# PaddlePaddle/Parakeet

Hardware: NVIDIA H100
Metric: audio-samples/sec (higher is better)
Workload: dtype bf16x3 (split-bf16 operands, fp32 accumulate; fp32-grade, 1e-3 parity)

## Files before the change

### parakeet_b200/csrc/pwg.cu

```cuda
#include <stdlib.h>
#include <string.h>

#include <algorithm>

#include "pk_host.h"
#include "pk_sm90.cuh"

namespace pk {

constexpr int kPwgR = 64;
constexpr int kPwgG = 128;
constexpr int kPwgS = 64;
constexpr int kPwgStages = 2;
constexpr int kPwgTile = 128 * kSwizzleBytes;
constexpr int kPwgStageBytes = 4 * kPwgTile;
constexpr int kPwgW2Bytes = 2 * kPwgTile;
constexpr int kPwgSmem = kPwgStages * kPwgStageBytes + kPwgW2Bytes + 1024 + 256;
static_assert(kPwgSmem <= 227 * 1024, "shared memory budget");
constexpr int kPwgConsumerThreads = 256;
constexpr int kPwgThreads = kPwgConsumerThreads + 128;
constexpr int kPwgG1Chunks = 5;

struct PwgLayerArgs {
  int batch, t, dil, aux_ch;
// ... 353 lines not shown
      }
      if (c_hi) {
        uint4 h, l;
        split8(v, h, l);
        const long long o = (static_cast<long long>(b) * T + t) * aux + g * 8;
        *reinterpret_cast<uint4*>(c_hi + o) = h;
        *reinterpret_cast<uint4*>(c_lo + o) = l;
      }
    }
  }
}

__global__ void pwg_first_conv_kernel(const float* __restrict__ noise, const float* __restrict__ w, const float* __restrict__ bias,
                                      const int32_t* __restrict__ lens, int t_len, long long total_rows,
                                      __nv_bfloat16* __restrict__ x_hi, __nv_bfloat16* __restrict__ x_lo) {
  const long long n = total_rows * 8;
  for (long long idx = blockIdx.x * static_cast<long long>(blockDim.x) + threadIdx.x; idx < n;
       idx += static_cast<long long>(gridDim.x) * blockDim.x) {
    const long long row = idx >> 3;
    const int g = idx & 7;
    const int b = row / t_len, t = row % t_len;
    const bool live = lens == nullptr || t < __ldg(lens + b);
    const float xv = __ldg(noise + row);
    float v[8];
#pragma unroll
    for (int e = 0; e < 8; ++e) v[e] = live ? fmaf(__ldg(w + g * 8 + e), xv, __ldg(bias + g * 8 + e)) : 0.f;
    uint4 h, l;
    split8(v, h, l);
    reinterpret_cast<uint4*>(x_hi)[idx] = h;
    reinterpret_cast<uint4*>(x_lo)[idx] = l;
  }
}

__global__ void __launch_bounds__(128)
pwg_tail_kernel(const float* __restrict__ skip, const float* __restrict__ skip_bias ,
                const float* __restrict__ w1 , const float* __restrict__ b1,
                const float* __restrict__ w2 , const float* __restrict__ b2, float scale, long long rows,
                float* __restrict__ out) {
  __shared__ float4 sw1[16 * 64];
  __shared__ float sb1[64], sw2[64], ssb[64];
  for (int i = threadIdx.x; i < 64 * 16; i += blockDim.x) {
    const int o = i >> 4, kq = i & 15;
    sw1[kq * 64 + o] = reinterpret_cast<const float4*>(w1)[i];
  }
  if (threadIdx.x < 64) {
    sb1[threadIdx.x] = b1[threadIdx.x];
    sw2[threadIdx.x] = w2[threadIdx.x];
    ssb[threadIdx.x] = skip_bias ? skip_bias[threadIdx.x] : 0.f;
  }
  __syncthreads();
  const float bias2 = __ldg(b2);
  const long long pairs = (rows + 1) >> 1;
  for (long long pr = blockIdx.x * static_cast<long long>(blockDim.x) + threadIdx.x; pr < pairs;
       pr += static_cast<long long>(gridDim.x) * blockDim.x) {
    const long long r0 = pr, r1 = pr + pairs;
    const bool has1 = r1 < rows;
    const float4* p0 = reinterpret_cast<const float4*>(skip + r0 * 64);
    const float4* p1 = reinterpret_cast<const float4*>(skip + (has1 ? r1 : r0) * 64);
    float h0[64], h1[64];
#pragma unroll
    for (int o = 0; o < 64; ++o) { h0[o] = sb1[o]; h1[o] = sb1[o]; }
#pragma unroll 1
    for (int kc = 0; kc < 4; ++kc) {
      float s0[16], s1[16];
#pragma unroll
      for (int q = 0; q < 4; ++q) {
        const float4 u = __ldg(p0 + kc * 4 + q), v = __ldg(p1 + kc * 4 + q);
        const float* sbp = ssb + kc * 16 + q * 4;
        s0[4 * q] = fmaxf((u.x + sbp[0]) * scale, 0.f); s0[4 * q + 1] = fmaxf((u.y + sbp[1]) * scale, 0.f);
        s0[4 * q + 2] = fmaxf((u.z + sbp[2]) * scale, 0.f); s0[4 * q + 3] = fmaxf((u.w + sbp[3]) * scale, 0.f);
        s1[4 * q] = fmaxf((v.x + sbp[0]) * scale, 0.f); s1[4 * q + 1] = fmaxf((v.y + sbp[1]) * scale, 0.f);
        s1[4 * q + 2] = fmaxf((v.z + sbp[2]) * scale, 0.f); s1[4 * q + 3] = fmaxf((v.w + sbp[3]) * scale, 0.f);
      }
#pragma unroll
      for (int q = 0; q < 4; ++q) {
#pragma unroll
        for (int o = 0; o < 64; ++o) {
          const float4 w = sw1[(kc * 4 + q) * 64 + o];
          h0[o] = fmaf(w.x, s0[4 * q], h0[o]); h0[o] = fmaf(w.y, s0[4 * q + 1], h0[o]);
          h0[o] = fmaf(w.z, s0[4 * q + 2], h0[o]); h0[o] = fmaf(w.w, s0[4 * q + 3], h0[o]);
          h1[o] = fmaf(w.x, s1[4 * q], h1[o]); h1[o] = fmaf(w.y, s1[4 * q + 1], h1[o]);
          h1[o] = fmaf(w.z, s1[4 * q + 2], h1[o]); h1[o] = fmaf(w.w, s1[4 * q + 3], h1[o]);
        }
      }
    }
    float y0 = bias2, y1 = bias2;
#pragma unroll
    for (int o = 0; o < 64; ++o) {
      y0 = fmaf(sw2[o], fmaxf(h0[o], 0.f), y0);
      y1 = fmaf(sw2[o], fmaxf(h1[o], 0.f), y1);
    }
    out[r0] = y0;
    if (has1) out[r1] = y1;
  }
}

}

extern "C" int pk_pwg_residual_layer(const pk_pwg_layer_args* a, pk_stream_t stream) {
  PK_CHECK_ARG(a != nullptr, "args is NULL");
// ... 93 lines not shown
  const size_t smem = floats * sizeof(float);
  PK_CHECK_ARG(smem <= 200 * 1024, "upsample tile does not fit shared memory (%zu bytes)", smem);
  static size_t attr_smem = 0;
  if (smem > attr_smem) {
    PK_CHECK_CUDA(cudaFuncSetAttribute(pwg_upsample_kernel, cudaFuncAttributeMaxDynamicSharedMemorySize, static_cast<int>(smem)));
    attr_smem = smem;
  }
  dim3 grid(frames, batch);
  pwg_upsample_kernel<<<grid, 256, smem, st>>>(conv_in_ws, frame_lens, a, c_f32, static_cast<__nv_bfloat16*>(c_hi),
                                               static_cast<__nv_bfloat16*>(c_lo));
  PK_CHECK_CUDA(cudaGetLastError());
  count_launch();
  return PK_OK;
}

extern "C" int pk_pwg_first_conv(const float* noise, const float* w, const float* bias, const int32_t* lens, int32_t batch,
                                 int32_t t, void* x_hi, void* x_lo, pk_stream_t stream) {
  PK_CHECK_ARG(noise && w && bias && x_hi && x_lo, "NULL pointer");
  PK_CHECK_ARG(batch > 0 && t > 0, "bad sizes");
  const long long rows = static_cast<long long>(batch) * t;
  const int threads = 256;
  const int blocks = static_cast<int>(std::min<long long>((rows * 8 + threads - 1) / threads, pk::sm_count() * 16LL));
  pk::pwg_first_conv_kernel<<<blocks, threads, 0, static_cast<cudaStream_t>(stream)>>>(
      noise, w, bias, lens, t, rows, static_cast<__nv_bfloat16*>(x_hi), static_cast<__nv_bfloat16*>(x_lo));
  PK_CHECK_CUDA(cudaGetLastError());
  pk::count_launch();
  return PK_OK;
}

extern "C" int pk_pwg_tail(const float* skip, const float* skip_bias, const float* w1, const float* b1, const float* w2,
                           const float* b2, float scale, int64_t rows, float* out, pk_stream_t stream) {
  PK_CHECK_ARG(skip && w1 && b1 && w2 && b2 && out, "NULL pointer");
  PK_CHECK_ARG(rows > 0, "bad sizes");
  const int threads = 128;
  const long long pairs = (rows + 1) / 2;
  const int blocks = static_cast<int>(std::min<long long>((pairs + threads - 1) / threads, pk::sm_count() * 12LL));
  pk::pwg_tail_kernel<<<blocks, threads, 0, static_cast<cudaStream_t>(stream)>>>(skip, skip_bias, w1, b1, w2, b2, scale, rows, out);
  PK_CHECK_CUDA(cudaGetLastError());
  pk::count_launch();
  return PK_OK;
}
```

### parakeet_b200/csrc/pk_sm90.cuh

```cuda
#pragma once
#include <cuda.h>
#include <cuda_bf16.h>
#include <cuda_runtime.h>
#include <stdint.h>

namespace pk {

constexpr int kSwizzleBytes = 128;
constexpr int kChunkK = 64;

__device__ __forceinline__ uint32_t smem_u32(const void* p) {
  return static_cast<uint32_t>(__cvta_generic_to_shared(p));
}

__device__ __forceinline__ void fence_barrier_init() {
  asm volatile("fence.mbarrier_init.release.cluster;" ::: "memory");
}

__device__ __forceinline__ void fence_proxy_async_all() { asm volatile("fence.proxy.async;" ::: "memory"); }

__device__ __forceinline__ void tma_prefetch_desc(const CUtensorMap* tm) {
  asm volatile("prefetch.tensormap [%0];" ::"l"(reinterpret_cast<uint64_t>(tm)) : "memory");
}

constexpr int kWgmmaK = 16;

__device__ __forceinline__ uint64_t make_smem_desc_sw128(uint32_t smem_addr) {
  uint64_t d = 0;
  d |= static_cast<uint64_t>((smem_addr & 0x3FFFFu) >> 4);
  d |= static_cast<uint64_t>(1) << 16;
  d |= static_cast<uint64_t>(1024 >> 4) << 32;
  d |= static_cast<uint64_t>(1) << 62;
  return d;
}
__device__ __forceinline__ uint64_t desc_kstep(int k) { return static_cast<uint64_t>((k * kWgmmaK * 2) >> 4); }
__device__ __forceinline__ uint64_t make_smem_desc_sw32(uint32_t smem_addr) {
  uint64_t d = 0;
  d |= static_cast<uint64_t>((smem_addr & 0x3FFFFu) >> 4);
  d |= static_cast<uint64_t>(1) << 16;
  d |= static_cast<uint64_t>(256 >> 4) << 32;
  d |= static_cast<uint64_t>(3) << 62;
  return d;
}

__device__ __forceinline__ void wgmma_fence() { asm volatile("wgmma.fence.sync.aligned;" ::: "memory"); }
__device__ __forceinline__ void wgmma_commit() { asm volatile("wgmma.commit_group.sync.aligned;" ::: "memory"); }
template <int N>
__device__ __forceinline__ void wgmma_wait() { asm volatile("wgmma.wait_group.sync.aligned %0;" ::"n"(N) : "memory"); }
template <int R>
__device__ __forceinline__ void reg_fence(float (&d)[R]) {
#pragma unroll
  for (int i = 0; i < R; ++i) asm volatile("" : "+f"(d[i])::"memory");
// ... 44 lines not shown
  asm volatile("{\n.reg .pred p;\nsetp.ne.b32 p, %101, 0;\n"
               "wgmma.mma_async.sync.aligned.m64n192k16.f32.bf16.bf16 {" PK_D96 "}, {%96,%97,%98,%99}, %100, p, 1, 1, 0;\n}\n"
               : PK_F32(0), PK_F32(32), PK_F32(64) : "r"(a[0]), "r"(a[1]), "r"(a[2]), "r"(a[3]), "l"(bdesc), "r"(accumulate));
}
#undef PK_F32
#undef PK_F8

__device__ __forceinline__ void split_bf16(float v, __nv_bfloat16& hi, __nv_bfloat16& lo) {
  hi = __float2bfloat16_rn(v);
  lo = __float2bfloat16_rn(v - __bfloat162float(hi));
}
__device__ __forceinline__ uint32_t pack_bf16x2(__nv_bfloat16 a, __nv_bfloat16 b) {
  return static_cast<uint32_t>(__bfloat16_as_ushort(a)) | (static_cast<uint32_t>(__bfloat16_as_ushort(b)) << 16);
}
__device__ __forceinline__ void split8(const float* v, uint4& hi, uint4& lo) {
  __nv_bfloat16 h[8], l[8];
#pragma unroll
  for (int i = 0; i < 8; ++i) split_bf16(v[i], h[i], l[i]);
  hi = make_uint4(pack_bf16x2(h[0], h[1]), pack_bf16x2(h[2], h[3]), pack_bf16x2(h[4], h[5]), pack_bf16x2(h[6], h[7]));
  lo = make_uint4(pack_bf16x2(l[0], l[1]), pack_bf16x2(l[2], l[3]), pack_bf16x2(l[4], l[5]), pack_bf16x2(l[6], l[7]));
}


__device__ __forceinline__ float4 lds_f4(uint32_t addr) {
  float4 v;
  asm volatile("ld.shared.v4.f32 {%0, %1, %2, %3}, [%4];" : "=f"(v.x), "=f"(v.y), "=f"(v.z), "=f"(v.w) : "r"(addr));
  return v;
}
__device__ __forceinline__ uint32_t lds_u32(uint32_t addr) {
  uint32_t v;
  asm volatile("ld.shared.u32 %0, [%1];" : "=r"(v) : "r"(addr) : "memory");
  return v;
}
__device__ __forceinline__ void sts_u32(uint32_t addr, uint32_t v) {
  asm volatile("st.shared.u32 [%0], %1;" ::"r"(addr), "r"(v) : "memory");
}

__device__ __forceinline__ void mbar_init_a(uint32_t bar, uint32_t count) {
  asm volatile("mbarrier.init.shared::cta.b64 [%0], %1;" ::"r"(bar), "r"(count) : "memory");
}
__device__ __forceinline__ void mbar_arrive_expect_tx_a(uint32_t bar, uint32_t bytes) {
  asm volatile("mbarrier.arrive.expect_tx.shared::cta.b64 _, [%0], %1;" ::"r"(bar), "r"(bytes) : "memory");
}
__device__ __forceinline__ void mbar_arrive_a(uint32_t bar) {
  asm volatile("mbarrier.arrive.shared::cta.b64 _, [%0];" ::"r"(bar) : "memory");
}
__device__ __forceinline__ void mbar_wait_a(uint32_t bar, uint32_t parity) {
  uint32_t ok = 0;
  for (uint32_t spin = 0; spin < (1u << 26); ++spin) {
    asm volatile(
        "{\n"
        ".reg .pred p;\n"
        "mbarrier.try_wait.parity.shared::cta.b64 p, [%1], %2;\n"
        "selp.u32 %0, 1, 0, p;\n"
        "}\n"
        : "=r"(ok)
        : "r"(bar), "r"(parity)
        : "memory");
    if (ok) return;
  }
  __trap();
}
__device__ __forceinline__ void tma_load_3d_a(uint32_t smem_dst, const CUtensorMap* tm, uint32_t bar, int c0, int c1, int c2) {
  asm volatile(
      "cp.async.bulk.tensor.3d.shared::cluster.global.tile.mbarrier::complete_tx::bytes [%0], [%1, {%3, %4, %5}], [%2];"
      ::"r"(smem_dst), "l"(reinterpret_cast<uint64_t>(tm)), "r"(bar), "r"(c0), "r"(c1), "r"(c2)
      : "memory");
}
__device__ __forceinline__ void tma_load_4d_a(uint32_t smem_dst, const CUtensorMap* tm, uint32_t bar, int c0, int c1, int c2, int c3) {
  asm volatile(
      "cp.async.bulk.tensor.4d.shared::cluster.global.tile.mbarrier::complete_tx::bytes [%0], [%1, {%3, %4, %5, %6}], [%2];"
      ::"r"(smem_dst), "l"(reinterpret_cast<uint64_t>(tm)), "r"(bar), "r"(c0), "r"(c1), "r"(c2), "r"(c3)
      : "memory");
}
__device__ __forceinline__ void tma_store_4d_a(const CUtensorMap* tm, uint32_t smem_src, int c0, int c1, int c2, int c3) {
  asm volatile("cp.async.bulk.tensor.4d.global.shared::cta.bulk_group [%0, {%2, %3, %4, %5}], [%1];"
               ::"l"(reinterpret_cast<uint64_t>(tm)), "r"(smem_src), "r"(c0), "r"(c1), "r"(c2), "r"(c3)
               : "memory");
}
__device__ __forceinline__ void bulk_prefetch_l2(const void* gptr, uint32_t bytes) {
  asm volatile("cp.async.bulk.prefetch.L2.global [%0], %1;" ::"l"(reinterpret_cast<uint64_t>(gptr)), "r"(bytes) : "memory");
}
__device__ __forceinline__ void bulk_commit() { asm volatile("cp.async.bulk.commit_group;" ::: "memory"); }
template <int N>
__device__ __forceinline__ void bulk_wait_read() { asm volatile("cp.async.bulk.wait_group.read %0;" ::"n"(N) : "memory"); }


constexpr int kStageSlotBytes = 64 * 32 * 4;
__device__ __forceinline__ uint32_t stage_addr(uint32_t slot, int row, int col) {
  return slot + row * 128 + ((((col >> 2) ^ (row & 7)) << 4) | ((col & 3) << 2));
}
template <int R>
__device__ __forceinline__ void stage_store(uint32_t slot, const float (&d)[R], int C, int wg_thread) {
  const int w = wg_thread >> 5, lane = wg_thread & 31;
  const int r0 = 16 * w + (lane >> 2), c0 = 2 * (lane & 3);
#pragma unroll
  for (int jj = 0; jj < 4; ++jj) {
    const int j = 4 * C + jj;
    asm volatile("st.shared.v2.f32 [%0], {%1, %2};" ::"r"(stage_addr(slot, r0, 8 * jj + c0)), "f"(d[4 * j]), "f"(d[4 * j + 1]) : "memory");
    asm volatile("st.shared.v2.f32 [%0], {%1, %2};" ::"r"(stage_addr(slot, r0 + 8, 8 * jj + c0)), "f"(d[4 * j + 2]), "f"(d[4 * j + 3])
                 : "memory");
  }
}
__device__ __forceinline__ void stage_load_row(uint32_t slot, int row, float (&v)[32]) {
#pragma unroll
  for (int k = 0; k < 8; ++k) {
    const float4 x = lds_f4(slot + row * 128 + ((k ^ (row & 7)) << 4));
    v[4 * k] = x.x; v[4 * k + 1] = x.y; v[4 * k + 2] = x.z; v[4 * k + 3] = x.w;
  }
}

}
```

### parakeet_b200/csrc/pwg_fc.cu

```cuda
#include <stdlib.h>
#include <string.h>

#include <algorithm>

#include "pk_host.h"
#include "pk_sm90.cuh"

namespace pk {
namespace fc {

constexpr int kPwgR = 64;
constexpr int kPwgG = 128;
constexpr int kATile = 128 * kSwizzleBytes;
constexpr int kQTile = 64 * kSwizzleBytes;
constexpr int kConsumerThreads = 256;
constexpr int kThreads = kConsumerThreads + 128;
constexpr int kFcG1Chunks = 4;
constexpr int kFcStages = 6;
constexpr int kFcStageBytes = 2 * kQTile;
constexpr int kFcUBytes = 2 * 64 * 32;
constexpr int kFcPBytes = 2 * 128 * 32;
constexpr int kFcW1Bytes = 3 * 2 * kATile;
constexpr int kFcW2Bytes = 2 * kATile;
constexpr int kFcSmem = kFcW1Bytes + kFcW2Bytes + kFcStages * kFcStageBytes + 1024 + 256;
static_assert(kFcUBytes + kFcPBytes <= kFcStageBytes, "the conditioning operands share one ring stage");
static_assert(kFcSmem <= 227 * 1024, "shared memory budget");

struct FcLayerArgs {
  int batch, t, dil, hop;
  int u_period, u_start_row, u_end_base;
  int p_row0;
  const int32_t* lens;
  float gate_c[128];
  float out_b[64];
  float k_a, k_g;
  float* skip;
  int skip_init;
};

__device__ __forceinline__ float ex2_approx(float x) {
  float y;
  asm("ex2.approx.ftz.f32 %0, %1;" : "=f"(y) : "f"(x));
  return y;
}
__device__ __forceinline__ float rcp_approx(float x) {
  float y;
  asm("rcp.approx.ftz.f32 %0, %1;" : "=f"(y) : "f"(x));
  return y;
}
__device__ __forceinline__ void split2(float a, float b, uint32_t& hi, uint32_t& lo) {
  const __nv_bfloat162 h = __floats2bfloat162_rn(a, b);
  hi = *reinterpret_cast<const uint32_t*>(&h);
  const float ra = a - __uint_as_float(hi << 16);
  const float rb = b - __uint_as_float(hi & 0xffff0000u);
  const __nv_bfloat162 l = __floats2bfloat162_rn(ra, rb);
  lo = *reinterpret_cast<const uint32_t*>(&l);
}

struct FcTileIter {
  int idx, step, tiles_per_b, total, t;
  const int32_t* lens;
  __device__ FcTileIter(const FcLayerArgs& p)
      : idx(static_cast<int>(blockIdx.x) - static_cast<int>(gridDim.x)), step(gridDim.x),
        tiles_per_b((p.t + 255) >> 8), total(((p.t + 255) >> 8) * p.batch * 2), t(p.t), lens(p.lens) {}
  __device__ bool next(int& b, int& m0, int& half) {
    for (;;) {
      idx += step;
      if (idx >= total) return false;
      const int w = idx >> 1;
      half = idx & 1;
      b = w / tiles_per_b;
      m0 = (w % tiles_per_b) * 256;
      const int len = lens ? min(__ldg(lens + b), t) : t;
      if (m0 < len) return true;
    }
  }
};

__global__ void __launch_bounds__(kThreads, 1)
pwg_layer_fc_kernel(const __grid_constant__ CUtensorMap tm_x, const __grid_constant__ CUtensorMap tm_u,
                    const __grid_constant__ CUtensorMap tm_p,
                    const __grid_constant__ CUtensorMap tm_w1_hi, const __grid_constant__ CUtensorMap tm_w1_lo,
                    const __grid_constant__ CUtensorMap tm_w2_hi, const __grid_constant__ CUtensorMap tm_w2_lo,
                    const __grid_constant__ CUtensorMap tm_y, const FcLayerArgs p) {
  extern __shared__ uint8_t smem_raw[];
  const uint32_t smem = (smem_u32(smem_raw) + 1023u) & ~1023u;
  const uint32_t w1 = smem;
  const uint32_t w2 = w1 + kFcW1Bytes;
  const uint32_t ring = w2 + kFcW2Bytes;
  const uint32_t bars = ring + kFcStages * kFcStageBytes;
  const uint32_t full_bar = bars;
  const uint32_t empty_bar = full_bar + 8 * kFcStages;
  const uint32_t w_bar = empty_bar + 8 * kFcStages;

  const int warp = threadIdx.x >> 5;
  const int lane = threadIdx.x & 31;

  if (threadIdx.x == kConsumerThreads) {
    tma_prefetch_desc(&tm_x); tma_prefetch_desc(&tm_u); tma_prefetch_desc(&tm_p);
    tma_prefetch_desc(&tm_w1_hi); tma_prefetch_desc(&tm_w1_lo); tma_prefetch_desc(&tm_w2_hi); tma_prefetch_desc(&tm_w2_lo);
    tma_prefetch_desc(&tm_y);
    for (int s = 0; s < kFcStages; ++s) { mbar_init_a(full_bar + 8 * s, 1); mbar_init_a(empty_bar + 8 * s, 4); }
    mbar_init_a(w_bar, 1);
    fence_barrier_init();
  }
  __syncthreads();

  if (warp >= kConsumerThreads / 32) {
    setmaxnreg_dec<40>();
    if (warp == kConsumerThreads / 32 && lane == 0) {
      mbar_arrive_expect_tx_a(w_bar, kFcW1Bytes + kFcW2Bytes);
      for (int j = 0; j < 3; ++j) {
        tma_load_3d_a(w1 + j * 2 * kATile, &tm_w1_hi, w_bar, j * kChunkK, 0, 0);
        tma_load_3d_a(w1 + j * 2 * kATile + kATile, &tm_w1_lo, w_bar, j * kChunkK, 0, 0);
      }
      tma_load_3d_a(w2, &tm_w2_hi, w_bar, 0, 0, 0);
      tma_load_3d_a(w2 + kATile, &tm_w2_lo, w_bar, 0, 0, 0);
      uint32_t it = 0;
      FcTileIter ti(p);
      int b, m0, half;
      while (ti.next(b, m0, half)) {
        const int mh = m0 + 128 * half;
        const int len = p.lens ? min(__ldg(p.lens + b), p.t) : p.t;
        const int m1 = ((len - 128) >> 7) << 7;
        const int urow = mh == 0 ? p.u_start_row
                         : (mh + 128 > len - 128) ? p.u_end_base + 384 * b + min(mh - m1, 256)
                                                  : mh % p.u_period;
        const int j0 = (m0 / p.hop - 2) & ~7;
        for (int wg = 0; wg < 2; ++wg) {
          const int rows = min(64, p.t - (mh + 64 * wg));
          if (!p.skip_init && rows > 0)
            bulk_prefetch_l2(p.skip + (static_cast<long long>(b) * p.t + mh + 64 * wg) * 64, rows * 64 * 4);
          for (int j = 0; j < kFcG1Chunks; ++j, ++it) {
            const int s = it % kFcStages;
            mbar_wait_a(empty_bar + 8 * s, ((it / kFcStages) & 1) ^ 1);
            const uint32_t st = ring + s * kFcStageBytes;
            const uint32_t fb = full_bar + 8 * s;
            if (j == 2) {
              mbar_arrive_expect_tx_a(fb, kFcUBytes + kFcPBytes);
              tma_load_4d_a(st, &tm_u, fb, 0, urow + 64 * wg, 0, 0);
              tma_load_4d_a(st + kFcUBytes, &tm_p, fb, j0, p.p_row0, b, 0);
            } else {
              mbar_arrive_expect_tx_a(fb, kFcStageBytes);
              const int wj = j == 0 ? 0 : j == 1 ? 2 : 1;
              tma_load_4d_a(st, &tm_x, fb, 0, mh + 64 * wg + (wj - 1) * p.dil, b, 0);
            }
          }
        }
      }
    }
  } else {
    setmaxnreg_inc<232>();
    const int wg = warp >> 2;
    const int rl = 16 * (warp & 3) + (lane >> 2);
    const int cq = 2 * (lane & 3);
    const float kSqrtHalf = 0.70710678118654752440f;
    mbar_wait_a(w_bar, 0);
    uint32_t it = wg * kFcG1Chunks;
    FcTileIter ti(p);
    int b, m0, half;
    bool more = ti.next(b, m0, half);
    bool first = true;
    while (more) {
      const int mh = m0 + 128 * half;
      float acc1[64], acc2[64];
      if (wg == 1 || !first) named_bar_sync(1 + wg, kConsumerThreads);
      first = false;
#pragma unroll
      for (int j = 0; j < kFcG1Chunks; ++j) {
        const int s = (it + j) % kFcStages;
        mbar_wait_a(full_bar + 8 * s, ((it + j) / kFcStages) & 1);
        const uint32_t st = ring + s * kFcStageBytes;
        wgmma_fence();
        if (j == 2) {
          const uint64_t a_hi = make_smem_desc_sw32(st), a_lo = make_smem_desc_sw32(st + kFcUBytes / 2);
          const uint64_t b_hi = make_smem_desc_sw32(st + kFcUBytes), b_lo = make_smem_desc_sw32(st + kFcUBytes + kFcPBytes / 2);
          wgmma_ss_n128(acc1, a_hi, b_hi, 1);
          wgmma_ss_n128(acc1, a_lo, b_hi, 1);
          wgmma_ss_n128(acc1, a_hi, b_lo, 1);
        } else {
          const int wj = j == 0 ? 0 : j == 1 ? 2 : 1;
          const uint64_t a_hi = make_smem_desc_sw128(st), a_lo = make_smem_desc_sw128(st + kQTile);
          const uint64_t b_hi = make_smem_desc_sw128(w1 + wj * 2 * kATile), b_lo = make_smem_desc_sw128(w1 + wj * 2 * kATile + kATile);
#pragma unroll
          for (int k = 0; k < 4; ++k) {
            wgmma_ss_n128(acc1, a_hi + desc_kstep(k), b_hi + desc_kstep(k), !(j == 0 && k == 0));
            wgmma_ss_n128(acc1, a_lo + desc_kstep(k), b_hi + desc_kstep(k), 1);
            wgmma_ss_n128(acc1, a_hi + desc_kstep(k), b_lo + desc_kstep(k), 1);
          }
        }
        wgmma_commit();
        if (j == kFcG1Chunks - 1) {
#pragma unroll
          for (int jj = 0; jj < 8; ++jj) {
#pragma unroll
            for (int hh = 0; hh < 2; ++hh) {
              const int r = rl + 8 * hh;
              const uint32_t off = r * kSwizzleBytes + ((((8 * jj + cq) >> 3) ^ (r & 7)) << 4) + (cq & 7) * 2;
              const uint32_t xh = lds_u32(st + off), xl = lds_u32(st + kQTile + off);
              acc2[4 * jj + 2 * hh] = 0.f;
              acc2[4 * jj + 2 * hh + 1] = 0.f;
              acc2[32 + 4 * jj + 2 * hh] = __uint_as_float(xh << 16) + __uint_as_float(xl << 16);
              acc2[32 + 4 * jj + 2 * hh + 1] = __uint_as_float(xh & 0xffff0000u) + __uint_as_float(xl & 0xffff0000u);
            }
          }
        }
        if (j > 0) {
          wgmma_wait<1>();
          __syncwarp();
          if (lane == 0) mbar_arrive_a(empty_bar + 8 * ((it + j - 1) % kFcStages));
        }
      }
      wgmma_wait<0>();
      reg_fence(acc1);
      const int cs = (it + kFcG1Chunks - 1) % kFcStages;
      const uint32_t ystage = ring + cs * kFcStageBytes;
      it += 2 * kFcG1Chunks;
      int nb, nm0, nhalf;
      const bool next = ti.next(nb, nm0, nhalf);
      if (wg == 0 || next) named_bar_arrive(2 - wg, kConsumerThreads);
      uint32_t zh[16], zl[16];
#pragma unroll
      for (int jj = 0; jj < 8; ++jj) {
        float z[4];
#pragma unroll
        for (int e = 0; e < 4; ++e) {
          const int c = 8 * jj + cq + (e & 1);
          const float e1 = ex2_approx(fminf(fmaf(acc1[4 * jj + e], p.k_a, p.gate_c[c]), 60.f));
          const float e2 = ex2_approx(fmaf(acc1[32 + 4 * jj + e], p.k_g, p.gate_c[64 + c]));
          const float t1 = 1.f + e1;
          z[e] = (1.f - e1) * rcp_approx(fmaf(t1, e2, t1));
        }
        split2(z[0], z[1], zh[2 * jj], zl[2 * jj]);
        split2(z[2], z[3], zh[2 * jj + 1], zl[2 * jj + 1]);
      }
      const uint64_t b2_hi = make_smem_desc_sw128(w2), b2_lo = make_smem_desc_sw128(w2 + kATile);
      wgmma_fence();
#pragma unroll
      for (int k = 0; k < 4; ++k) {
        const uint32_t ah[4] = {zh[4 * k], zh[4 * k + 1], zh[4 * k + 2], zh[4 * k + 3]};
        const uint32_t al[4] = {zl[4 * k], zl[4 * k + 1], zl[4 * k + 2], zl[4 * k + 3]};
        wgmma_rs_n128(acc2, ah, b2_hi + desc_kstep(k), 1);
        wgmma_rs_n128(acc2, al, b2_hi + desc_kstep(k), 1);
        wgmma_rs_n128(acc2, ah, b2_lo + desc_kstep(k), 1);
      }
      wgmma_commit();
      wgmma_wait<0>();
      reg_fence(acc2);
      const int len = p.lens ? min(__ldg(p.lens + b), p.t) : p.t;
#pragma unroll
      for (int hh = 0; hh < 2; ++hh) {
        const int r = rl + 8 * hh;
        const bool live = mh + wg * 64 + r < len;
#pragma unroll
        for (int jj = 0; jj < 8; ++jj) {
          const int c = 8 * jj + cq;
          const float y0 = live ? (acc2[32 + 4 * jj + 2 * hh] + p.out_b[c]) * kSqrtHalf : 0.f;
          const float y1 = live ? (acc2[32 + 4 * jj + 2 * hh + 1] + p.out_b[c + 1]) * kSqrtHalf : 0.f;
          uint32_t oh, ol;
          split2(y0, y1, oh, ol);
          const uint32_t off = r * kSwizzleBytes + (((c >> 3) ^ (r & 7)) << 4) + (cq & 7) * 2;
          sts_u32(ystage + off, oh);
          sts_u32(ystage + kQTile + off, ol);
        }
      }
      fence_proxy_async_all();
      named_bar_sync(3 + wg, 128);
      const bool store_lane = (threadIdx.x & 127) == 0;
      if (store_lane) {
        tma_store_4d_a(&tm_y, ystage, 0, mh + wg * 64, b, 0);
        bulk_commit();
      }
#pragma unroll
      for (int hh = 0; hh < 2; ++hh) {
        const int trow = mh + wg * 64 + rl + 8 * hh;
        if (trow < p.t) {
          const long long row_off = (static_cast<long long>(b) * p.t + trow) * 64;
#pragma unroll
          for (int jj = 0; jj < 8; ++jj) {
            float* d2 = p.skip + row_off + 8 * jj + cq;
            const float s0 = acc2[4 * jj + 2 * hh], s1 = acc2[4 * jj + 2 * hh + 1];
            if (p.skip_init) *reinterpret_cast<float2*>(d2) = make_float2(s0, s1);
            else asm volatile("red.global.add.v2.f32 [%0], {%1, %2};" ::"l"(d2), "f"(s0), "f"(s1) : "memory");
          }
        }
      }
      if (store_lane) {
        bulk_wait_read<0>();
#pragma unroll
        for (int w = 0; w < 4; ++w) mbar_arrive_a(empty_bar + 8 * cs);
      }
      b = nb; m0 = nm0; half = nhalf; more = next;
    }
  }
}

}
}

extern "C" int pk_pwg_residual_layer_fc(const pk_pwg_layer_fc_args* a, pk_stream_t stream) {
  using namespace pk;
  using namespace pk::fc;
  PK_CHECK_ARG(a != nullptr, "args is NULL");
  PK_CHECK_ARG(a->batch > 0 && a->t > 0 && a->dilation >= 1 && a->hop >= 256, "bad batch/t/dilation/hop (hop must be >= 256)");
  PK_CHECK_ARG(a->x_hi && a->x_lo && a->y_hi && a->y_lo && a->u_hi && a->u_lo && a->p_hi && a->p_lo && a->w1_hi && a->w1_lo &&
               a->w2_hi && a->w2_lo && a->bias1 && a->bias2 && a->skip, "NULL pointer in pk_pwg_layer_fc_args");
  PK_CHECK_ARG(a->x_hi != a->y_hi, "layer output must not alias its input");
  PK_CHECK_ARG(a->u_period > 0 && (a->u_period % 128) == 0 && a->u_start_row >= a->u_period && a->u_end_base >= a->u_start_row + 128 &&
               a->u_rows >= a->u_end_base + 384 * a->batch, "bad compact band table layout");
  PK_CHECK_ARG(a->p_rows > 0 && a->p_row0 >= 0 && a->p_row0 + 128 <= a->p_rows && (a->p_ld % 8) == 0 && a->p_ld >= 64 && a->p_frames > 0 &&
               a->p_frames <= a->p_ld, "bad P plane geometry");
  CUtensorMap tx, tu, tp, tw1_hi, tw1_lo, tw2_hi, tw2_lo, ty;
  int rc;
  const uint64_t T = a->t, B = a->batch;
  if ((rc = encode_tmap_bf16_planes(&tx, a->x_hi, a->x_lo, kPwgR, T, B, kPwgR, T * kPwgR, 64))) return rc;
  if ((rc = encode_tmap_bf16_planes(&ty, a->y_hi, a->y_lo, kPwgR, T, B, kPwgR, T * kPwgR, 64))) return rc;
  if ((rc = encode_tmap_bf16_planes(&tu, a->u_hi, a->u_lo, 64, a->u_rows, 1, 64, 0, 64, 16))) return rc;
  const uint64_t prow = a->p_rows, pld = a->p_ld;
  if ((rc = encode_tmap_bf16_planes(&tp, a->p_hi, a->p_lo, pld, prow, B, pld, prow * pld, 128, 16))) return rc;
  const uint64_t k1 = 5 * kChunkK;
  if ((rc = encode_tmap_bf16_3d(&tw1_hi, a->w1_hi, 3 * kChunkK, kPwgG, 1, k1, k1 * kPwgG, 128))) return rc;
  if ((rc = encode_tmap_bf16_3d(&tw1_lo, a->w1_lo, 3 * kChunkK, kPwgG, 1, k1, k1 * kPwgG, 128))) return rc;
  if ((rc = encode_tmap_bf16_3d(&tw2_hi, a->w2_hi, 64, 128, 1, 64, 0, 128))) return rc;
  if ((rc = encode_tmap_bf16_3d(&tw2_lo, a->w2_lo, 64, 128, 1, 64, 0, 128))) return rc;
  static bool attr_set = false;
  if (!attr_set) {
    PK_CHECK_CUDA(cudaFuncSetAttribute(pwg_layer_fc_kernel, cudaFuncAttributeMaxDynamicSharedMemorySize, kFcSmem));
    attr_set = true;
  }
  FcLayerArgs p;
  p.batch = a->batch; p.t = a->t; p.dil = a->dilation; p.hop = a->hop;
  p.u_period = a->u_period; p.u_start_row = a->u_start_row; p.u_end_base = a->u_end_base;
  p.p_row0 = a->p_row0;
  p.lens = a->lens; p.skip = a->skip; p.skip_init = a->skip_init;
  constexpr float kLog2e = 1.4426950408889634f;
  p.k_a = -2.f * kLog2e; p.k_g = -kLog2e;
  for (int i = 0; i < 64; ++i) {
    p.gate_c[i] = -2.f * kLog2e * a->bias1[i];
    p.gate_c[64 + i] = -kLog2e * a->bias1[64 + i];
    p.out_b[i] = a->bias2[64 + i];
  }
  const cudaStream_t st = static_cast<cudaStream_t>(stream);
  const int tiles = ((a->t + 255) / 256) * 2 * a->batch;
  const int grid = std::min(tiles, sm_count());
  pwg_layer_fc_kernel<<<grid, kThreads, kFcSmem, static_cast<cudaStream_t>(stream)>>>(tx, tu, tp, tw1_hi, tw1_lo, tw2_hi, tw2_lo, ty, p);
  PK_CHECK_CUDA(cudaGetLastError());
  count_launch();
  return PK_OK;
}
```

Baseline: 65.48 million.

## Double-buffer skip loads in PWG tail kernel via cp.async

The tail kernel now stages each thread's skip-row chunks into a per-thread double-buffered shared-memory area using cp.async. It prefetches the next k-chunk, or the next row pair's first chunk, while the current one is computed. This is meant to hide global load latency behind the FMA-heavy inner loop. The cost is 32KB of extra dynamic shared memory per block, which may reduce occupancy, plus the added wait and commit bookkeeping.

Measured after the change: 65.50 million (median of 6 runs). About the same (+0.0%).

```diff
diff --git a/parakeet_b200/csrc/pwg.cu b/parakeet_b200/csrc/pwg.cu
--- a/parakeet_b200/csrc/pwg.cu
+++ b/parakeet_b200/csrc/pwg.cu
@@ -409,13 +409,24 @@
   }
 }
 
-__global__ void __launch_bounds__(128)
+constexpr int kTailThreads = 128;
+constexpr int kTailStageBytes = 2 * 8 * kTailThreads * 16;
+
+__device__ __forceinline__ void cp_async16(uint32_t smem_dst, const void* gsrc) {
+  asm volatile("cp.async.cg.shared.global [%0], [%1], 16;" ::"r"(smem_dst), "l"(gsrc) : "memory");
+}
+__device__ __forceinline__ void cp_async_commit() { asm volatile("cp.async.commit_group;" ::: "memory"); }
+template <int N>
+__device__ __forceinline__ void cp_async_wait() { asm volatile("cp.async.wait_group %0;" ::"n"(N) : "memory"); }
+
+__global__ void __launch_bounds__(kTailThreads)
 pwg_tail_kernel(const float* __restrict__ skip, const float* __restrict__ skip_bias ,
                 const float* __restrict__ w1 , const float* __restrict__ b1,
                 const float* __restrict__ w2 , const float* __restrict__ b2, float scale, long long rows,
                 float* __restrict__ out) {
   __shared__ float4 sw1[16 * 64];
   __shared__ float sb1[64], sw2[64], ssb[64];
+  extern __shared__ float4 tail_stage[];
   for (int i = threadIdx.x; i < 64 * 16; i += blockDim.x) {
     const int o = i >> 4, kq = i & 15;
     sw1[kq * 64 + o] = reinterpret_cast<const float4*>(w1)[i];
@@ -428,21 +439,41 @@
   __syncthreads();
   const float bias2 = __ldg(b2);
   const long long pairs = (rows + 1) >> 1;
-  for (long long pr = blockIdx.x * static_cast<long long>(blockDim.x) + threadIdx.x; pr < pairs;
-       pr += static_cast<long long>(gridDim.x) * blockDim.x) {
+  const long long first = blockIdx.x * static_cast<long long>(blockDim.x) + threadIdx.x;
+  const long long stride = static_cast<long long>(gridDim.x) * blockDim.x;
+  const uint32_t slot0 = smem_u32(tail_stage) + threadIdx.x * 16, slot_stride = kTailThreads * 16;
+  auto fetch = [&](long long pr, int kc, int buf) {
+    const long long r0 = pr, r1 = pr + pairs;
+    const float4* p0 = reinterpret_cast<const float4*>(skip + r0 * 64) + kc * 4;
+    const float4* p1 = reinterpret_cast<const float4*>(skip + (r1 < rows ? r1 : r0) * 64) + kc * 4;
+#pragma unroll
+    for (int q = 0; q < 4; ++q) {
+      cp_async16(slot0 + (buf * 8 + q) * slot_stride, p0 + q);
+      cp_async16(slot0 + (buf * 8 + 4 + q) * slot_stride, p1 + q);
+    }
+    cp_async_commit();
+  };
+  if (first < pairs) fetch(first, 0, 0);
+  int buf = 0;
+  for (long long pr = first; pr < pairs; pr += stride) {
     const long long r0 = pr, r1 = pr + pairs;
     const bool has1 = r1 < rows;
-    const float4* p0 = reinterpret_cast<const float4*>(skip + r0 * 64);
-    const float4* p1 = reinterpret_cast<const float4*>(skip + (has1 ? r1 : r0) * 64);
     float h0[64], h1[64];
 #pragma unroll
     for (int o = 0; o < 64; ++o) { h0[o] = sb1[o]; h1[o] = sb1[o]; }
 #pragma unroll 1
-    for (int kc = 0; kc < 4; ++kc) {
+    for (int kc = 0; kc < 4; ++kc, buf ^= 1) {
+      const bool more = kc < 3 || pr + stride < pairs;
+      if (more) {
+        fetch(kc < 3 ? pr : pr + stride, (kc + 1) & 3, buf ^ 1);
+        cp_async_wait<1>();
+      } else {
+        cp_async_wait<0>();
+      }
       float s0[16], s1[16];
 #pragma unroll
       for (int q = 0; q < 4; ++q) {
-        const float4 u = __ldg(p0 + kc * 4 + q), v = __ldg(p1 + kc * 4 + q);
+        const float4 u = lds_f4(slot0 + (buf * 8 + q) * slot_stride), v = lds_f4(slot0 + (buf * 8 + 4 + q) * slot_stride);
         const float* sbp = ssb + kc * 16 + q * 4;
         s0[4 * q] = fmaxf((u.x + sbp[0]) * scale, 0.f); s0[4 * q + 1] = fmaxf((u.y + sbp[1]) * scale, 0.f);
         s0[4 * q + 2] = fmaxf((u.z + sbp[2]) * scale, 0.f); s0[4 * q + 3] = fmaxf((u.w + sbp[3]) * scale, 0.f);
@@ -602,10 +633,16 @@
                            const float* b2, float scale, int64_t rows, float* out, pk_stream_t stream) {
   PK_CHECK_ARG(skip && w1 && b1 && w2 && b2 && out, "NULL pointer");
   PK_CHECK_ARG(rows > 0, "bad sizes");
-  const int threads = 128;
+  const int threads = pk::kTailThreads;
   const long long pairs = (rows + 1) / 2;
   const int blocks = static_cast<int>(std::min<long long>((pairs + threads - 1) / threads, pk::sm_count() * 12LL));
-  pk::pwg_tail_kernel<<<blocks, threads, 0, static_cast<cudaStream_t>(stream)>>>(skip, skip_bias, w1, b1, w2, b2, scale, rows, out);
+  static bool attr_set = false;
+  if (!attr_set) {
+    PK_CHECK_CUDA(cudaFuncSetAttribute(pk::pwg_tail_kernel, cudaFuncAttributeMaxDynamicSharedMemorySize, pk::kTailStageBytes));
+    attr_set = true;
+  }
+  pk::pwg_tail_kernel<<<blocks, threads, pk::kTailStageBytes, static_cast<cudaStream_t>(stream)>>>(skip, skip_bias, w1, b1, w2, b2,
+                                                                                                 scale, rows, out);
   PK_CHECK_CUDA(cudaGetLastError());
   pk::count_launch();
   return PK_OK;
```

## Store layer output directly from registers and permute W2 rows at load

Applied to the files above, without the earlier changes.

The TMA store of the y output through a shared-memory ring stage is replaced by direct 16-byte global stores from registers. The W2 weights are loaded by consumer threads with a row permutation, so each thread's accumulator columns become contiguous, which allows vectorised v4 shared loads of the residual and v4 skip stores and reductions. The ring stage is therefore released right after the GEMM instead of after the bulk store drains. The cost is more register pressure and uncoalesced-ish per-thread global stores, and the row permutation must match the wgmma fragment layout exactly.

After: 45.96 million before, 47.81 million after, median of 6. +4.0%, better.

```diff
diff --git a/parakeet_b200/csrc/pk_sm90.cuh b/parakeet_b200/csrc/pk_sm90.cuh
--- a/parakeet_b200/csrc/pk_sm90.cuh
+++ b/parakeet_b200/csrc/pk_sm90.cuh
@@ -18,6 +18,7 @@
 }
 
 __device__ __forceinline__ void fence_proxy_async_all() { asm volatile("fence.proxy.async;" ::: "memory"); }
+__device__ __forceinline__ void fence_proxy_async_shared() { asm volatile("fence.proxy.async.shared::cta;" ::: "memory"); }
 
 __device__ __forceinline__ void tma_prefetch_desc(const CUtensorMap* tm) {
   asm volatile("prefetch.tensormap [%0];" ::"l"(reinterpret_cast<uint64_t>(tm)) : "memory");
@@ -128,8 +129,16 @@
   asm volatile("ld.shared.u32 %0, [%1];" : "=r"(v) : "r"(addr) : "memory");
   return v;
 }
+__device__ __forceinline__ uint4 lds_u4(uint32_t addr) {
+  uint4 v;
+  asm volatile("ld.shared.v4.b32 {%0, %1, %2, %3}, [%4];" : "=r"(v.x), "=r"(v.y), "=r"(v.z), "=r"(v.w) : "r"(addr) : "memory");
+  return v;
+}
 __device__ __forceinline__ void sts_u32(uint32_t addr, uint32_t v) {
   asm volatile("st.shared.u32 [%0], %1;" ::"r"(addr), "r"(v) : "memory");
+}
+__device__ __forceinline__ void sts_u4(uint32_t addr, uint4 v) {
+  asm volatile("st.shared.v4.b32 [%0], {%1, %2, %3, %4};" ::"r"(addr), "r"(v.x), "r"(v.y), "r"(v.z), "r"(v.w) : "memory");
 }
 
 __device__ __forceinline__ void mbar_init_a(uint32_t bar, uint32_t count) {
@@ -169,17 +178,9 @@
       ::"r"(smem_dst), "l"(reinterpret_cast<uint64_t>(tm)), "r"(bar), "r"(c0), "r"(c1), "r"(c2), "r"(c3)
       : "memory");
 }
-__device__ __forceinline__ void tma_store_4d_a(const CUtensorMap* tm, uint32_t smem_src, int c0, int c1, int c2, int c3) {
-  asm volatile("cp.async.bulk.tensor.4d.global.shared::cta.bulk_group [%0, {%2, %3, %4, %5}], [%1];"
-               ::"l"(reinterpret_cast<uint64_t>(tm)), "r"(smem_src), "r"(c0), "r"(c1), "r"(c2), "r"(c3)
-               : "memory");
-}
 __device__ __forceinline__ void bulk_prefetch_l2(const void* gptr, uint32_t bytes) {
   asm volatile("cp.async.bulk.prefetch.L2.global [%0], %1;" ::"l"(reinterpret_cast<uint64_t>(gptr)), "r"(bytes) : "memory");
 }
-__device__ __forceinline__ void bulk_commit() { asm volatile("cp.async.bulk.commit_group;" ::: "memory"); }
-template <int N>
-__device__ __forceinline__ void bulk_wait_read() { asm volatile("cp.async.bulk.wait_group.read %0;" ::"n"(N) : "memory"); }
 
 
 constexpr int kStageSlotBytes = 64 * 32 * 4;
diff --git a/parakeet_b200/csrc/pwg_fc.cu b/parakeet_b200/csrc/pwg_fc.cu
--- a/parakeet_b200/csrc/pwg_fc.cu
+++ b/parakeet_b200/csrc/pwg_fc.cu
@@ -34,9 +34,18 @@
   float gate_c[128];
   float out_b[64];
   float k_a, k_g;
+  const uint4* w2_hi;
+  const uint4* w2_lo;
+  __nv_bfloat16* y_hi;
+  __nv_bfloat16* y_lo;
   float* skip;
   int skip_init;
 };
+
+__device__ __forceinline__ int w2_source_row(int n) {
+  const int jj = (n & 63) >> 3, q = (n >> 1) & 3, e = n & 1;
+  return n < 64 ? 16 * (jj >> 1) + 4 * q + 2 * (jj & 1) + e : 64 + 32 * (jj >> 2) + 8 * q + 2 * (jj & 3) + e;
+}
 
 __device__ __forceinline__ float ex2_approx(float x) {
   float y;
@@ -81,8 +90,7 @@
 pwg_layer_fc_kernel(const __grid_constant__ CUtensorMap tm_x, const __grid_constant__ CUtensorMap tm_u,
                     const __grid_constant__ CUtensorMap tm_p,
                     const __grid_constant__ CUtensorMap tm_w1_hi, const __grid_constant__ CUtensorMap tm_w1_lo,
-                    const __grid_constant__ CUtensorMap tm_w2_hi, const __grid_constant__ CUtensorMap tm_w2_lo,
-                    const __grid_constant__ CUtensorMap tm_y, const FcLayerArgs p) {
+                    const FcLayerArgs p) {
   extern __shared__ uint8_t smem_raw[];
   const uint32_t smem = (smem_u32(smem_raw) + 1023u) & ~1023u;
   const uint32_t w1 = smem;
@@ -98,8 +106,7 @@
 
   if (threadIdx.x == kConsumerThreads) {
     tma_prefetch_desc(&tm_x); tma_prefetch_desc(&tm_u); tma_prefetch_desc(&tm_p);
-    tma_prefetch_desc(&tm_w1_hi); tma_prefetch_desc(&tm_w1_lo); tma_prefetch_desc(&tm_w2_hi); tma_prefetch_desc(&tm_w2_lo);
-    tma_prefetch_desc(&tm_y);
+    tma_prefetch_desc(&tm_w1_hi); tma_prefetch_desc(&tm_w1_lo);
     for (int s = 0; s < kFcStages; ++s) { mbar_init_a(full_bar + 8 * s, 1); mbar_init_a(empty_bar + 8 * s, 4); }
     mbar_init_a(w_bar, 1);
     fence_barrier_init();
@@ -109,13 +116,11 @@
   if (warp >= kConsumerThreads / 32) {
     setmaxnreg_dec<40>();
     if (warp == kConsumerThreads / 32 && lane == 0) {
-      mbar_arrive_expect_tx_a(w_bar, kFcW1Bytes + kFcW2Bytes);
+      mbar_arrive_expect_tx_a(w_bar, kFcW1Bytes);
       for (int j = 0; j < 3; ++j) {
         tma_load_3d_a(w1 + j * 2 * kATile, &tm_w1_hi, w_bar, j * kChunkK, 0, 0);
         tma_load_3d_a(w1 + j * 2 * kATile + kATile, &tm_w1_lo, w_bar, j * kChunkK, 0, 0);
       }
-      tma_load_3d_a(w2, &tm_w2_hi, w_bar, 0, 0, 0);
-      tma_load_3d_a(w2 + kATile, &tm_w2_lo, w_bar, 0, 0, 0);
       uint32_t it = 0;
       FcTileIter ti(p);
       int b, m0, half;
@@ -153,8 +158,17 @@
     setmaxnreg_inc<232>();
     const int wg = warp >> 2;
     const int rl = 16 * (warp & 3) + (lane >> 2);
-    const int cq = 2 * (lane & 3);
+    const int q = lane & 3;
     const float kSqrtHalf = 0.70710678118654752440f;
+#pragma unroll
+    for (int k = 0; k < 2 * 128 * 8 / kConsumerThreads; ++k) {
+      const int i = threadIdx.x + k * kConsumerThreads;
+      const int plane = i >> 10, n = (i >> 3) & 127, k8 = i & 7;
+      const uint4 v = __ldg((plane ? p.w2_lo : p.w2_hi) + w2_source_row(n) * 8 + k8);
+      sts_u4(w2 + plane * kATile + n * kSwizzleBytes + ((k8 ^ (n & 7)) << 4), v);
+    }
+    fence_proxy_async_all();
+    named_bar_sync(3, kConsumerThreads);
     mbar_wait_a(w_bar, 0);
     uint32_t it = wg * kFcG1Chunks;
     FcTileIter ti(p);
@@ -192,16 +206,21 @@
         wgmma_commit();
         if (j == kFcG1Chunks - 1) {
 #pragma unroll
-          for (int jj = 0; jj < 8; ++jj) {
-#pragma unroll
-            for (int hh = 0; hh < 2; ++hh) {
-              const int r = rl + 8 * hh;
-              const uint32_t off = r * kSwizzleBytes + ((((8 * jj + cq) >> 3) ^ (r & 7)) << 4) + (cq & 7) * 2;
-              const uint32_t xh = lds_u32(st + off), xl = lds_u32(st + kQTile + off);
-              acc2[4 * jj + 2 * hh] = 0.f;
-              acc2[4 * jj + 2 * hh + 1] = 0.f;
-              acc2[32 + 4 * jj + 2 * hh] = __uint_as_float(xh << 16) + __uint_as_float(xl << 16);
-              acc2[32 + 4 * jj + 2 * hh + 1] = __uint_as_float(xh & 0xffff0000u) + __uint_as_float(xl & 0xffff0000u);
+          for (int i = 0; i < 32; ++i) acc2[i] = 0.f;
+#pragma unroll
+          for (int hh = 0; hh < 2; ++hh) {
+            const int r = rl + 8 * hh;
+#pragma unroll
+            for (int g = 0; g < 2; ++g) {
+              const uint32_t off = r * kSwizzleBytes + (((4 * g + q) ^ (r & 7)) << 4);
+              const uint4 h4 = lds_u4(st + off), l4 = lds_u4(st + kQTile + off);
+              const uint32_t xh[4] = {h4.x, h4.y, h4.z, h4.w}, xl[4] = {l4.x, l4.y, l4.z, l4.w};
+#pragma unroll
+              for (int u = 0; u < 4; ++u) {
+                const int jj = 4 * g + u;
+                acc2[32 + 4 * jj + 2 * hh] = __uint_as_float(xh[u] << 16) + __uint_as_float(xl[u] << 16);
+                acc2[32 + 4 * jj + 2 * hh + 1] = __uint_as_float(xh[u] & 0xffff0000u) + __uint_as_float(xl[u] & 0xffff0000u);
+              }
             }
           }
         }
@@ -213,8 +232,9 @@
       }
       wgmma_wait<0>();
       reg_fence(acc1);
-      const int cs = (it + kFcG1Chunks - 1) % kFcStages;
-      const uint32_t ystage = ring + cs * kFcStageBytes;
+      fence_proxy_async_shared();
+      __syncwarp();
+      if (lane == 0) mbar_arrive_a(empty_bar + 8 * ((it + kFcG1Chunks - 1) % kFcStages));
       it += 2 * kFcG1Chunks;
       int nb, nm0, nhalf;
       const bool next = ti.next(nb, nm0, nhalf);
@@ -225,7 +245,7 @@
         float z[4];
 #pragma unroll
         for (int e = 0; e < 4; ++e) {
-          const int c = 8 * jj + cq + (e & 1);
+          const int c = 8 * jj + 2 * q + (e & 1);
           const float e1 = ex2_approx(fminf(fmaf(acc1[4 * jj + e], p.k_a, p.gate_c[c]), 60.f));
           const float e2 = ex2_approx(fmaf(acc1[32 + 4 * jj + e], p.k_g, p.gate_c[64 + c]));
           const float t1 = 1.f + e1;
@@ -250,45 +270,38 @@
       const int len = p.lens ? min(__ldg(p.lens + b), p.t) : p.t;
 #pragma unroll
       for (int hh = 0; hh < 2; ++hh) {
-        const int r = rl + 8 * hh;
-        const bool live = mh + wg * 64 + r < len;
-#pragma unroll
-        for (int jj = 0; jj < 8; ++jj) {
-          const int c = 8 * jj + cq;
-          const float y0 = live ? (acc2[32 + 4 * jj + 2 * hh] + p.out_b[c]) * kSqrtHalf : 0.f;
-          const float y1 = live ? (acc2[32 + 4 * jj + 2 * hh + 1] + p.out_b[c + 1]) * kSqrtHalf : 0.f;
-          uint32_t oh, ol;
-          split2(y0, y1, oh, ol);
-          const uint32_t off = r * kSwizzleBytes + (((c >> 3) ^ (r & 7)) << 4) + (cq & 7) * 2;
-          sts_u32(ystage + off, oh);
-          sts_u32(ystage + kQTile + off, ol);
-        }
-      }
-      fence_proxy_async_all();
-      named_bar_sync(3 + wg, 128);
-      const bool store_lane = (threadIdx.x & 127) == 0;
-      if (store_lane) {
-        tma_store_4d_a(&tm_y, ystage, 0, mh + wg * 64, b, 0);
-        bulk_commit();
-      }
-#pragma unroll
-      for (int hh = 0; hh < 2; ++hh) {
         const int trow = mh + wg * 64 + rl + 8 * hh;
         if (trow < p.t) {
           const long long row_off = (static_cast<long long>(b) * p.t + trow) * 64;
-#pragma unroll
-          for (int jj = 0; jj < 8; ++jj) {
-            float* d2 = p.skip + row_off + 8 * jj + cq;
-            const float s0 = acc2[4 * jj + 2 * hh], s1 = acc2[4 * jj + 2 * hh + 1];
-            if (p.skip_init) *reinterpret_cast<float2*>(d2) = make_float2(s0, s1);
-            else asm volatile("red.global.add.v2.f32 [%0], {%1, %2};" ::"l"(d2), "f"(s0), "f"(s1) : "memory");
-          }
-        }
-      }
-      if (store_lane) {
-        bulk_wait_read<0>();
-#pragma unroll
-        for (int w = 0; w < 4; ++w) mbar_arrive_a(empty_bar + 8 * cs);
+          const bool live = trow < len;
+#pragma unroll
+          for (int g = 0; g < 2; ++g) {
+            uint32_t oh[4], ol[4];
+#pragma unroll
+            for (int u = 0; u < 4; ++u) {
+              const int jj = 4 * g + u, c = 32 * g + 8 * q + 2 * u;
+              const float y0 = live ? (acc2[32 + 4 * jj + 2 * hh] + p.out_b[c]) * kSqrtHalf : 0.f;
+              const float y1 = live ? (acc2[32 + 4 * jj + 2 * hh + 1] + p.out_b[c + 1]) * kSqrtHalf : 0.f;
+              split2(y0, y1, oh[u], ol[u]);
+            }
+            const long long off = row_off + 32 * g + 8 * q;
+            asm volatile("st.global.v4.b32 [%0], {%1, %2, %3, %4};" ::"l"(p.y_hi + off), "r"(oh[0]), "r"(oh[1]), "r"(oh[2]),
+                         "r"(oh[3]) : "memory");
+            asm volatile("st.global.v4.b32 [%0], {%1, %2, %3, %4};" ::"l"(p.y_lo + off), "r"(ol[0]), "r"(ol[1]), "r"(ol[2]),
+                         "r"(ol[3]) : "memory");
+          }
+#pragma unroll
+          for (int m = 0; m < 4; ++m) {
+            float* d = p.skip + row_off + 16 * m + 4 * q;
+            const float s0 = acc2[8 * m + 2 * hh], s1 = acc2[8 * m + 2 * hh + 1];
+            const float s2 = acc2[8 * m + 4 + 2 * hh], s3 = acc2[8 * m + 4 + 2 * hh + 1];
+            if (p.skip_init)
+              asm volatile("st.global.v4.f32 [%0], {%1, %2, %3, %4};" ::"l"(d), "f"(s0), "f"(s1), "f"(s2), "f"(s3) : "memory");
+            else
+              asm volatile("red.global.add.v4.f32 [%0], {%1, %2, %3, %4};" ::"l"(d), "f"(s0), "f"(s1), "f"(s2), "f"(s3)
+                           : "memory");
+          }
+        }
       }
       b = nb; m0 = nm0; half = nhalf; more = next;
     }
@@ -310,19 +323,19 @@
                a->u_rows >= a->u_end_base + 384 * a->batch, "bad compact band table layout");
   PK_CHECK_ARG(a->p_rows > 0 && a->p_row0 >= 0 && a->p_row0 + 128 <= a->p_rows && (a->p_ld % 8) == 0 && a->p_ld >= 64 && a->p_frames > 0 &&
                a->p_frames <= a->p_ld, "bad P plane geometry");
-  CUtensorMap tx, tu, tp, tw1_hi, tw1_lo, tw2_hi, tw2_lo, ty;
+  PK_CHECK_ARG(((reinterpret_cast<uintptr_t>(a->y_hi) | reinterpret_cast<uintptr_t>(a->y_lo) | reinterpret_cast<uintptr_t>(a->skip) |
+                 reinterpret_cast<uintptr_t>(a->w2_hi) | reinterpret_cast<uintptr_t>(a->w2_lo)) & 15) == 0,
+               "y, skip and w2 planes must be 16-byte aligned");
+  CUtensorMap tx, tu, tp, tw1_hi, tw1_lo;
   int rc;
   const uint64_t T = a->t, B = a->batch;
   if ((rc = encode_tmap_bf16_planes(&tx, a->x_hi, a->x_lo, kPwgR, T, B, kPwgR, T * kPwgR, 64))) return rc;
-  if ((rc = encode_tmap_bf16_planes(&ty, a->y_hi, a->y_lo, kPwgR, T, B, kPwgR, T * kPwgR, 64))) return rc;
   if ((rc = encode_tmap_bf16_planes(&tu, a->u_hi, a->u_lo, 64, a->u_rows, 1, 64, 0, 64, 16))) return rc;
   const uint64_t prow = a->p_rows, pld = a->p_ld;
   if ((rc = encode_tmap_bf16_planes(&tp, a->p_hi, a->p_lo, pld, prow, B, pld, prow * pld, 128, 16))) return rc;
   const uint64_t k1 = 5 * kChunkK;
   if ((rc = encode_tmap_bf16_3d(&tw1_hi, a->w1_hi, 3 * kChunkK, kPwgG, 1, k1, k1 * kPwgG, 128))) return rc;
   if ((rc = encode_tmap_bf16_3d(&tw1_lo, a->w1_lo, 3 * kChunkK, kPwgG, 1, k1, k1 * kPwgG, 128))) return rc;
-  if ((rc = encode_tmap_bf16_3d(&tw2_hi, a->w2_hi, 64, 128, 1, 64, 0, 128))) return rc;
-  if ((rc = encode_tmap_bf16_3d(&tw2_lo, a->w2_lo, 64, 128, 1, 64, 0, 128))) return rc;
   static bool attr_set = false;
   if (!attr_set) {
     PK_CHECK_CUDA(cudaFuncSetAttribute(pwg_layer_fc_kernel, cudaFuncAttributeMaxDynamicSharedMemorySize, kFcSmem));
@@ -333,6 +346,8 @@
   p.u_period = a->u_period; p.u_start_row = a->u_start_row; p.u_end_base = a->u_end_base;
   p.p_row0 = a->p_row0;
   p.lens = a->lens; p.skip = a->skip; p.skip_init = a->skip_init;
+  p.w2_hi = static_cast<const uint4*>(a->w2_hi); p.w2_lo = static_cast<const uint4*>(a->w2_lo);
+  p.y_hi = static_cast<__nv_bfloat16*>(a->y_hi); p.y_lo = static_cast<__nv_bfloat16*>(a->y_lo);
   constexpr float kLog2e = 1.4426950408889634f;
   p.k_a = -2.f * kLog2e; p.k_g = -kLog2e;
   for (int i = 0; i < 64; ++i) {
@@ -343,7 +358,7 @@
   const cudaStream_t st = static_cast<cudaStream_t>(stream);
   const int tiles = ((a->t + 255) / 256) * 2 * a->batch;
   const int grid = std::min(tiles, sm_count());
-  pwg_layer_fc_kernel<<<grid, kThreads, kFcSmem, static_cast<cudaStream_t>(stream)>>>(tx, tu, tp, tw1_hi, tw1_lo, tw2_hi, tw2_lo, ty, p);
+  pwg_layer_fc_kernel<<<grid, kThreads, kFcSmem, static_cast<cudaStream_t>(stream)>>>(tx, tu, tp, tw1_hi, tw1_lo, p);
   PK_CHECK_CUDA(cudaGetLastError());
   count_launch();
   return PK_OK;
```
